# EdwardLiuyc/StaticMapping

Measured on AMD Instinct MI355X. Metric: scan-pair alignments/sec (120k-pt KITTI-64, 20 ICP iters), higher is better.
Workload: dtype f32/f64; 1 GPU; BASELINE config #2: IcpFast point-to-plane, 120k-pt synthetic Velodyne-64 scan pair vs CalculateNormals target (~21695 pts), exactly 20 iterations, rho 0.7; 512 distinct consecutive pairs of a synthetic drive (speed 6-10 m/s, yaw rate +-0.2 rad/s, seed 5), guess = previous pair's motion; pairs_per_gpu=512, distinct_pairs=512, target_points_mean=21695, nn_mode=grid, guess=extrapolated, split_after=2, parallelism=pairs round-robin over 1 GPU(s), one RCCL gather of poses, rccl_ranks=1

## Files before the change

staticmapping_amd/csrc/icp_kernels.hip:

```cpp
#include <type_traits>
#include "smhip_device.h"
#include "kd_median_tree.h"
#include "grid_lookup.h"
#include "icp_tail_math.h"

namespace smhip {

__device__ __forceinline__ bool xcd_block(int nblk, int npairs, int b_pair_base, int& pair, int& blk) {
  const int id = blockIdx.x;
  const int j = id >> 3;
  const int local = (j / nblk) * 8 + (id & 7);
  pair = b_pair_base + local;
  blk = j % nblk;
  return local < npairs;
}

__global__ __launch_bounds__(256) void tgt_reduce(IcpDev b) {
  const int pair = b.pair_base + blockIdx.y;
  const int nt = b.in[pair].nt;
  const float4* tp = b.tgt_p + (size_t)pair * b.nt_cap;
  double sx = 0, sy = 0, sz = 0;
  float mn[3] = {INFINITY, INFINITY, INFINITY}, mx[3] = {-INFINITY, -INFINITY, -INFINITY};
  const int chunk = (nt + gridDim.x - 1) / gridDim.x;
  const int lo = blockIdx.x * chunk, hi = min(nt, lo + chunk);
// ... 485 lines not shown
__device__ __forceinline__ int wave_max_i(int v) {
  constexpr int kId = -0x7fffffff - 1;
  v = max(v, dpp_or<0x111, 0xf>(kId, v));
  v = max(v, dpp_or<0x112, 0xf>(kId, v));
  v = max(v, dpp_or<0x114, 0xf>(kId, v));
  v = max(v, dpp_or<0x118, 0xf>(kId, v));
  v = max(v, dpp_or<0x142, 0xa>(kId, v));
  v = max(v, dpp_or<0x143, 0xc>(kId, v));
  return __builtin_amdgcn_readlane(v, 63);
}

__device__ __forceinline__ void search_row(const uint2* __restrict__ words, const uint32_t* __restrict__ cstart,
                                           const float4* __restrict__ tq, int rowbase, int xa, int xb,
                                           float qx, float qy, float qz, Best& best);

__device__ __forceinline__ float search_radius2(float r2cap, float dub2, float margin) {
  const float r = sqrtf(dub2) + margin;
  return fminf(r2cap, r * r);
}
__device__ __forceinline__ float search_margin(float delta) { return fminf(fmaxf(3.0f * delta, 0.01f), 0.10f); }

__global__ __launch_bounds__(kNnThreads) void nn_ball(IcpDev b, int nblk) {
  int pair, blk;
  if (!xcd_block(nblk, b.npairs, b.pair_base, pair, blk)) return;
  PairState* st = &b.state[pair];
  if (st->done) return;
  const int count = st->ns;
  const int base0 = blk * (kNnThreads * kBallItems);
  if (base0 >= count) return;
  __shared__ uint32_t s_hist[kHistBins];
  for (int k = threadIdx.x; k < kHistBins; k += kNnThreads) s_hist[k] = 0;
  __syncthreads();
  const int lane = threadIdx.x & 63;
  const size_t so = (size_t)pair * b.ns_cap;
  const uint2* __restrict__ words = b.words + (size_t)pair * kMaxGridWords;
  const uint32_t* __restrict__ cstart = b.cstart + (size_t)pair * (b.nt_cap + 1);
  const float4* __restrict__ tq = b.tq + (size_t)pair * b.nt_cap;
  const float ox = st->origin[0], oy = st->origin[1], oz = st->origin[2];
  const float h = st->h, inv_h = st->inv_h;
  const int nx = st->nx, ny = st->ny, nz = st->nz, wx = st->wx;
  const float r2cap = st->rcap2;
  const bool have_prev = st->iter > 0;
  const Pot pot = {(float)st->pot_a, (float)st->pot_b, 0.f, 0.f};
  uint32_t min_lb = 0xffffffffu;

  for (int it = 0; it < kBallItems; ++it) {
    const int e = base0 + it * kNnThreads + threadIdx.x;
    bool hard = false;
    int i = -1;
    if (e < count) {
      i = e;
      double px, py, pz;
      const float4 s4 = ld_src(b, so + i);
      transform_point(st->M, s4, px, py, pz);
      const float qx = (float)px, qy = (float)py, qz = (float)pz;
      Best best = {INFINITY, -1, INFINITY};
      float d2out = INFINITY, lbout = 0.f;
      int jout = -1;
      if (isfinite(qx) && isfinite(qy) && isfinite(qz)) {
        float R2 = r2cap;
        int jp = -1;
        if (have_prev) {
          jp = b.idx[so + i];
          if (jp >= 0) {
            double ux, uy, uz;
            transform_point(st->M_prev, s4, ux, uy, uz);
            const float ex = qx - (float)ux, ey = qy - (float)uy, ez = qz - (float)uz;
            R2 = search_radius2(r2cap, dist2(tq[jp], qx, qy, qz), search_margin(sqrtf(fmaf(ez, ez, fmaf(ey, ey, ex * ex)))));
          }
        }
        const float Rs = sqrtf(R2) * 1.0001f + 1.0e-3f * h;
        const int x0 = max(cell_coord(qx - Rs, ox, inv_h), 0), x1 = min(cell_coord(qx + Rs, ox, inv_h), nx - 1);
        const int y0 = max(cell_coord(qy - Rs, oy, inv_h), 0), y1 = min(cell_coord(qy + Rs, oy, inv_h), ny - 1);
        const int z0 = max(cell_coord(qz - Rs, oz, inv_h), 0), z1 = min(cell_coord(qz + Rs, oz, inv_h), nz - 1);
        if (x0 <= x1) {
          const float slack = 2.0e-3f * h;
          for (int z = z0; z <= z1; ++z) {
            const float zl = oz + (float)z * h;
            const float dz = fmaxf(fmaxf(zl - qz, qz - (zl + h)) - slack, 0.f);
            for (int y = y0; y <= y1; ++y) {
              const float yl = oy + (float)y * h;
              const float dy = fmaxf(fmaxf(yl - qy, qy - (yl + h)) - slack, 0.f);
              if (fmaf(dy, dy, dz * dz) > R2) continue;
              uint32_t sb, se;
              row_slots(words, (z * ny + y) * wx, x0, x1, sb, se);
              if (se > sb) {
                const uint32_t j0 = cstart[sb], j1 = cstart[se];
                for (uint32_t j = j0; j < j1; ++j) test_ascending_ru(tq[j], (int)j, qx, qy, qz, best);
              }
            }
          }
        }
        if (best.d2 <= R2) {
          d2out = best.d2;
          jout = best.j;
          lbout = sqrtf(fminf(best.s2, R2));
        } else {
          d2out = R2;
          jout = best.j >= 0 ? best.j : jp;
          lbout = -sqrtf(R2);
          hard = true;
          min_lb = min(min_lb, __float_as_uint(R2));
        }
      }
      b.d2[so + i] = d2out;
      st_match(b, so + i, jout, with_pot(lbout, pot_at(pot, norm3(s4.x, s4.y, s4.z))));
      const uint32_t key = __float_as_uint(d2out);
      if (key < 0x7f800000u) atomicAdd(&s_hist[key >> kHistShift], 1u);
    }
    const unsigned long long hm = __ballot(hard);
    if (hm) {
      uint32_t basepos = 0;
      if (lane == 0) basepos = atomicAdd(&st->hard_count, (uint32_t)__popcll(hm));
      basepos = (uint32_t)__builtin_amdgcn_readlane((int)basepos, 0);
      if (hard) b.hlist[so + basepos + __popcll(hm & ((1ull << lane) - 1ull))] = i;
    }
  }
  if (min_lb != 0xffffffffu) atomicMin(&st->min_lb_key, min_lb);
  __syncthreads();
  uint32_t* gh = b.hist + (size_t)pair * kHistBins;
  for (int k = threadIdx.x; k < kHistBins; k += kNnThreads) {
    const uint32_t v = s_hist[k];
    if (v) atomicAdd(&gh[k], v);
  }
}


__device__ __forceinline__ int nabo_class(uint32_t buckets) { return buckets <= 2u ? 0 : (buckets <= 4u ? 1 : (buckets <= 7u ? 2 : 3)); }
__device__ __forceinline__ int32_t* nabo_list_slot(const IcpDev& b, size_t so, int c, uint32_t k) {
  int32_t* base = (c < 2 ? b.dlist : b.hlist) + so;
  return (c & 1) ? base + (b.ns_cap - 1) - k : base + k;
}

template <int ITEMS>
__device__ __forceinline__ void nabo_list_append(const IcpDev& b, PairState* st, size_t so, int base, int ns, uint32_t nabo_failed, int lane) {
  static_assert(ITEMS <= 32, "one bit per round");
  if (!__ballot(nabo_failed != 0u)) return;
  unsigned long long cls2 = 0;
#pragma unroll
  for (int it = 0; it < ITEMS; ++it) {
    const int i = base + it * kNnThreads + (int)threadIdx.x;
    const uint32_t w = (nabo_failed >> it) & 1u ? (uint32_t)b.nabo_work[so + min(i, ns - 1)] : 0u;
    cls2 |= (unsigned long long)nabo_class(w) << (2 * it);
  }
  uint32_t tot[4] = {0, 0, 0, 0};
  const unsigned long long lt = (1ull << lane) - 1ull;
  auto class_masks = [&](int it, unsigned long long* m) {
    const bool f = (nabo_failed >> it) & 1u;
    const uint32_t c = (uint32_t)(cls2 >> (2 * it)) & 3u;
    const unsigned long long fm = __ballot(f), b0 = __ballot(f && (c & 1u)), b1 = __ballot(f && (c & 2u));
    m[0] = fm & ~b0 & ~b1; m[1] = fm & b0 & ~b1; m[2] = fm & ~b0 & b1; m[3] = fm & b0 & b1;
    return fm;
  };
#pragma unroll
  for (int it = 0; it < ITEMS; ++it) {
    unsigned long long m[4];
    if (!class_masks(it, m)) continue;
#pragma unroll
    for (int c = 0; c < 4; ++c) tot[c] += (uint32_t)__popcll(m[c]);
  }
  uint32_t basepos[4];
#pragma unroll
  for (int c = 0; c < 4; ++c) {
    uint32_t v = 0;
    if (lane == 0 && tot[c]) v = atomicAdd(&st->nabo_count[c], tot[c]);
    basepos[c] = (uint32_t)__builtin_amdgcn_readlane((int)v, 0);
  }
#pragma unroll
  for (int it = 0; it < ITEMS; ++it) {
    unsigned long long m[4];
    if (!class_masks(it, m)) continue;
    const uint32_t c = (uint32_t)(cls2 >> (2 * it)) & 3u;
    if ((nabo_failed >> it) & 1u) {
      const unsigned long long mine = c == 0 ? m[0] : (c == 1 ? m[1] : (c == 2 ? m[2] : m[3]));
      const uint32_t bp = c == 0 ? basepos[0] : (c == 1 ? basepos[1] : (c == 2 ? basepos[2] : basepos[3]));
      *nabo_list_slot(b, so, (int)c, bp + (uint32_t)__popcll(mine & lt)) = base + it * kNnThreads + (int)threadIdx.x;
    }
#pragma unroll
    for (int c2 = 0; c2 < 4; ++c2) basepos[c2] += (uint32_t)__popcll(m[c2]);
  }
}

template <int ITEMS, bool NABO = false>
__global__ __launch_bounds__(kNnThreads) void nn_certify(IcpDev b, int nblk) {
  int pair, blk;
  if (!xcd_block(nblk, b.npairs, b.pair_base, pair, blk)) return;
  PairState* st = &b.state[pair];
  if (st->done) return;
  const int ns = st->ns;
  const int base = blk * (kNnThreads * ITEMS);
  if (base >= ns) return;
  double Mc[12];
#pragma unroll
  for (int k = 0; k < 12; ++k) Mc[k] = st->M[k];
  const Pot pot = {(float)st->pot_a, (float)st->pot_b, 0.f, 0.f};
  __shared__ uint32_t s_hist[kHistBins];
  for (int k = threadIdx.x; k < kHistBins; k += kNnThreads) s_hist[k] = 0;
  __syncthreads();
  const int lane = threadIdx.x & 63;
  const size_t so = (size_t)pair * b.ns_cap;
  const float4* __restrict__ tq = b.tq + (size_t)pair * b.nt_cap;
  const float r_need = 0.9f * sqrtf(st->rcap2);
  uint32_t min_lb = 0xffffffffu;
  uint32_t nabo_failed = 0;
  int ic = min(base + (int)threadIdx.x, ns - 1);
  float4 s_1 = ld_src(b, so + ic);
  float l_1 = ld_lb(b, so + ic);
  int j_1 = b.idx[so + ic];
  ic = min(base + kNnThreads + (int)threadIdx.x, ns - 1);
  float4 s_2 = ld_src(b, so + ic);
  float l_2 = ld_lb(b, so + ic);
  int j_2 = b.idx[so + ic];
  float4 t_1 = tq[max(j_1, 0)];
  for (int it = 0; it < ITEMS; ++it) {
    const int i = base + it * kNnThreads + threadIdx.x;
    bool hard = false, fail = false;
    const float4 s = s_1;
    const float l = l_1;
    const int j = j_1;
    const float4 t = t_1;
    s_1 = s_2; l_1 = l_2; j_1 = j_2;
    if (it + 1 < ITEMS) t_1 = tq[max(j_1, 0)];
    if (it + 2 < ITEMS) {
      ic = min(i + 2 * kNnThreads, ns - 1);
      s_2 = ld_src(b, so + ic);
      l_2 = ld_lb(b, so + ic);
      j_2 = b.idx[so + ic];
    }
    if (i < ns) {
      double px, py, pz;
      transform_point(Mc, s, px, py, pz);
      const float qx = (float)px, qy = (float)py, qz = (float)pz;
      const float Lp = bound_now(l, pot_at(pot, norm3(s.x, s.y, s.z)));
      fail = true;
      if (NABO) {
        const float Pn = pot_at(pot, norm3(s.x, s.y, s.z));
        if (isfinite(qx) && isfinite(qy) && isfinite(qz) && l > 0.f && j >= 0 &&
            l - Pn - 4.0e-7f * (l + Pn) - 1.3e-7f * (fabsf(qx) + fabsf(qy) + fabsf(qz)) > 0.f) {
          const float d1 = dist2(t, qx, qy, qz);
          b.d2[so + i] = d1;
          atomicAdd(&s_hist[__float_as_uint(d1) >> kHistShift], 1u);
          fail = false;
        }
      } else if (isfinite(qx) && isfinite(qy) && isfinite(qz) && Lp > 0.f) {
        if (l > 0.f && j >= 0) {
          const float d1 = dist2(t, qx, qy, qz);
          if (d1 < Lp * Lp) {
            b.d2[so + i] = d1;
            atomicAdd(&s_hist[__float_as_uint(d1) >> kHistShift], 1u);
            fail = false;
          }
        } else if (l < 0.f && Lp >= r_need) {
          const float lb2 = Lp * Lp;
          b.d2[so + i] = lb2;
          atomicAdd(&s_hist[__float_as_uint(lb2) >> kHistShift], 1u);
          min_lb = min(min_lb, __float_as_uint(lb2));
          hard = true;
          fail = false;
        }
      }
    }
    const unsigned long long dm = __ballot(fail);
    if (NABO) {
      if (fail) nabo_failed |= 1u << it;
    } else if (dm) {
      uint32_t basepos = 0;
      if (lane == 0) basepos = atomicAdd(&st->deferred_count, (uint32_t)__popcll(dm));
      basepos = (uint32_t)__builtin_amdgcn_readlane((int)basepos, 0);
      if (fail) b.dlist[so + basepos + __popcll(dm & ((1ull << lane) - 1ull))] = i;
    }
    const unsigned long long hm = __ballot(hard);
    if (hm) {
      uint32_t basepos = 0;
      if (lane == 0) basepos = atomicAdd(&st->hard_count, (uint32_t)__popcll(hm));
      basepos = (uint32_t)__builtin_amdgcn_readlane((int)basepos, 0);
      if (hard) b.hlist[so + basepos + __popcll(hm & ((1ull << lane) - 1ull))] = i;
    }
  }
  if (NABO) nabo_list_append<ITEMS>(b, st, so, base, ns, nabo_failed, lane);
#pragma unroll
  for (int off = 32; off > 0; off >>= 1) min_lb = min(min_lb, (uint32_t)__shfl_xor((int)min_lb, off, 64));
  if (lane == 0 && min_lb != 0xffffffffu) atomicMin(&st->min_lb_key, min_lb);
  __syncthreads();
  uint32_t* gh = b.hist + (size_t)pair * kHistBins;
  for (int k = threadIdx.x; k < kHistBins; k += kNnThreads) {
    const uint32_t v = s_hist[k];
    if (v) atomicAdd(&gh[k], v);
  }
}

__device__ __forceinline__ void sweep_run(const float4* __restrict__ tq, uint32_t j0, uint32_t j1,
                                          float qx, float qy, float qz, Best& best) {
  uint32_t j = j0;
  for (; j + 4 <= j1; j += 4) {
    const float4 t0 = tq[j], t1 = tq[j + 1], t2 = tq[j + 2], t3 = tq[j + 3];
    test_ascending_ru(t0, (int)j, qx, qy, qz, best);
    test_ascending_ru(t1, (int)j + 1, qx, qy, qz, best);
    test_ascending_ru(t2, (int)j + 2, qx, qy, qz, best);
    test_ascending_ru(t3, (int)j + 3, qx, qy, qz, best);
  }
  for (; j < j1; ++j) test_ascending_ru(tq[j], (int)j, qx, qy, qz, best);
}

#ifndef SMHIP_PHASE_TIMING
#define SMHIP_PHASE_TIMING 0
#endif
#if SMHIP_PHASE_TIMING
#define SMHIP_PHASE(k) do { if (timing) { const unsigned long long now_ = __builtin_readcyclecounter(); tacc[k] += now_ - tprev; tprev = now_; } } while (0)
__device__ __forceinline__ unsigned long long* phase_counter(const IcpDev& b, int k) {
  return reinterpret_cast<unsigned long long*>(b.tpart) + (k / 7) * 16 + 9 + (k % 7);
}
#else
#define SMHIP_PHASE(k) do { } while (0)
#endif
template <int ITEMS, bool FIRST>
__device__ __forceinline__ void ball_lds_rounds(const IcpDev& b, PairState* st, const PairState* ls, int pair, int base0, const double* Mc,
                                                uint32_t* s_hist, uint32_t& min_lb) {
  const int ns = ls->ns;
  const Pot pot = {(float)ls->pot_a, (float)ls->pot_b, (float)ls->step_a, (float)ls->step_b};
  const float Mtx = (float)Mc[3], Mty = (float)Mc[7], Mtz = (float)Mc[11];
#if SMHIP_PHASE_TIMING
  const bool timing = (b.debug_flags & 16) != 0;
  unsigned long long tacc[14] = {0, 0, 0, 0, 0, 0, 0, 0, 0, 0, 0, 0, 0, 0};
  unsigned long long tprev = timing ? __builtin_readcyclecounter() : 0ull;
#endif
  __shared__ uint32_t s_tab[kLdsTableCap];
  __shared__ float4 s_pts[kLdsPointCap];
  __shared__ uint32_t s_roff[kLdsRowCap + 1];
  __shared__ uint32_t s_occ[kLdsRowCap / 32 + 1];
  __shared__ uint32_t s_w[17];
  __shared__ int s_box[2][6];
  float4* s_e = nullptr;
  uint16_t* s_slot = nullptr;
  uint32_t* s_nsearch = nullptr;
  if constexpr (!FIRST) {
    __shared__ float4 s_e_[ITEMS * kNnThreads];
    __shared__ uint16_t s_slot_[ITEMS * kNnThreads];
    __shared__ uint32_t s_nsearch_;
    s_e = s_e_; s_slot = s_slot_; s_nsearch = &s_nsearch_;
    if (threadIdx.x == 6) s_nsearch_ = 0;
  }
  if (threadIdx.x < 6) { s_box[0][threadIdx.x] = threadIdx.x < 3 ? 0x3fffffff : -0x3fffffff; s_box[1][threadIdx.x] = s_box[0][threadIdx.x]; }
  __syncthreads();
  const int lane = threadIdx.x & 63;
  const size_t so = (size_t)pair * b.ns_cap;
  const uint2* __restrict__ words = b.words + (size_t)pair * kMaxGridWords;
  const uint32_t* __restrict__ cstart = b.cstart + (size_t)pair * (b.nt_cap + 1);
  const float4* __restrict__ tq = b.tq + (size_t)pair * b.nt_cap;
  const float ox = ls->origin[0], oy = ls->origin[1], oz = ls->origin[2];
  const float h = ls->h, inv_h = ls->inv_h;
  const int nx = ls->nx, ny = ls->ny, nz = ls->nz, wx = ls->wx, nw = ls->nw;
  const float r2cap = ls->rcap2;
  const float r_need = 0.9f * sqrtf(r2cap);
  const bool have_prev = !FIRST && ls->iter > 0;
  const bool certify = have_prev && b.certify;

  int i = base0 + threadIdx.x;
  float4 s_cur = make_float4(0, 0, 0, 0);
  int jp_cur = -1;
  float l_cur = 0.f;
  if (i < ns) {
    s_cur = ld_src(b, so + i);
    if (have_prev) { jp_cur = b.idx[so + i]; if (certify) l_cur = ld_lb(b, so + i); }
  }

  auto query_round = [&](const int it, float& qx, float& qy, float& qz, bool& valid) -> bool {
    const int base = base0 + it * kNnThreads;
    if (base >= ns) return false;
    i = base + threadIdx.x;
    const int i_next = i + kNnThreads;
    float4 s_next = make_float4(0, 0, 0, 0);
    int jp_next = -1;
    float l_next = 0.f;
    if (it + 1 < ITEMS && i_next < ns) {
      s_next = ld_src(b, so + i_next);
      if (have_prev) { jp_next = b.idx[so + i_next]; if (certify) l_next = ld_lb(b, so + i_next); }
    }
    SMHIP_PHASE(0);
    qx = 0.f; qy = 0.f; qz = 0.f;
    valid = false;
    if (i < ns) {
      double px, py, pz;
      transform_point(Mc, s_cur, px, py, pz);
      qx = (float)px; qy = (float)py; qz = (float)pz;
      valid = isfinite(qx) && isfinite(qy) && isfinite(qz);
    }
    const bool has_jp = valid && jp_cur >= 0;
    float dub2 = INFINITY;
    if (has_jp) dub2 = dist2(tq[jp_cur], qx, qy, qz);
    bool need_search = valid, hard = false;
    if (i < ns && !valid) {
      b.d2[so + i] = INFINITY; st_match(b, so + i, -1, 0.f);
    }
    const float sn = __builtin_amdgcn_sqrtf(fmaf(s_cur.z, s_cur.z, fmaf(s_cur.y, s_cur.y, s_cur.x * s_cur.x)));
    const float delta = have_prev ? fmaf(pot.sa, sn, pot.sb) : 0.03f;
    if (certify && valid) {
      const float Lp = bound_now(l_cur, pot_at(pot, sn));
      if (Lp > 0.f) {
        if (l_cur > 0.f && has_jp && dub2 < Lp * Lp) {
          b.d2[so + i] = dub2;
          atomicAdd(&s_hist[__float_as_uint(dub2) >> kHistShift], 1u);
          need_search = false;
        } else if (l_cur < 0.f && Lp >= r_need) {
          const float lb2 = Lp * Lp;
          b.d2[so + i] = lb2;
          atomicAdd(&s_hist[__float_as_uint(lb2) >> kHistShift], 1u);
          min_lb = min(min_lb, __float_as_uint(lb2));
          hard = true;
          need_search = false;
        }
      }
    }
    if constexpr (!FIRST) {
      const unsigned long long sm = __ballot(need_search);
      if (sm) {
        uint32_t basepos = 0;
        if (lane == 0) basepos = atomicAdd(s_nsearch, (uint32_t)__popcll(sm));
        basepos = (uint32_t)__builtin_amdgcn_readlane((int)basepos, 0);
        if (need_search) {
          const uint32_t pos = basepos + __popcll(sm & ((1ull << lane) - 1ull));
          s_e[pos] = make_float4(qx, qy, qz, has_jp ? search_radius2(r2cap, dub2, search_margin(delta)) : r2cap);
          s_slot[pos] = (uint16_t)(it * kNnThreads + (int)threadIdx.x);
        }
      }
    }
    {
      const unsigned long long hm = __ballot(hard);
      if (hm) {
        uint32_t basepos = 0;
        if (lane == 0) basepos = atomicAdd(&st->hard_count, (uint32_t)__popcll(hm));
        basepos = (uint32_t)__builtin_amdgcn_readlane((int)basepos, 0);
        if (hard) b.hlist[so + basepos + __popcll(hm & ((1ull << lane) - 1ull))] = i;
      }
    }
    s_cur = s_next; jp_cur = jp_next; l_cur = l_next;
    SMHIP_PHASE(1);
    return true;
  };
  auto search_round = [&](const int sr, const bool mine, const bool wave_live, const float qx, const float qy, const float qz, const float R2, const int gi) {
    int* box = s_box[sr & 1];
#if SMHIP_PHASE_TIMING
    const unsigned long long tround = timing ? __builtin_readcyclecounter() : 0ull;
#endif
    int x0 = 1, x1 = 0, y0 = 1, y1 = 0, z0 = 1, z1 = 0;
    if (mine) {
      const float Rs = __builtin_amdgcn_sqrtf(R2) * 1.0001f + 1.0e-3f * h;
      x0 = max(cell_coord(qx - Rs, ox, inv_h), 0); x1 = min(cell_coord(qx + Rs, ox, inv_h), nx - 1);
      y0 = max(cell_coord(qy - Rs, oy, inv_h), 0); y1 = min(cell_coord(qy + Rs, oy, inv_h), ny - 1);
      z0 = max(cell_coord(qz - Rs, oz, inv_h), 0); z1 = min(cell_coord(qz + Rs, oz, inv_h), nz - 1);
    }
    const bool inbox = mine && x0 <= x1 && y0 <= y1 && z0 <= z1;
    if (wave_live) {
      const int big = 0x3fffffff;
      const int mx0 = wave_min_i(inbox ? x0 : big), mx1 = wave_max_i(inbox ? x1 : -big);
      const int my0 = wave_min_i(inbox ? y0 : big), my1 = wave_max_i(inbox ? y1 : -big);
      const int mz0 = wave_min_i(inbox ? z0 : big), mz1 = wave_max_i(inbox ? z1 : -big);
      if (lane == 0 && mx0 <= mx1) {
        atomicMin(&box[0], mx0); atomicMin(&box[1], my0); atomicMin(&box[2], mz0);
        atomicMax(&box[3], mx1); atomicMax(&box[4], my1); atomicMax(&box[5], mz1);
      }
    }
    SMHIP_PHASE(3);
    __syncthreads();
    const int X0 = box[0], Y0 = box[1], Z0 = box[2];
    const int nxl = box[3] - X0 + 2, nyl = box[4] - Y0 + 1, nzl = box[5] - Z0 + 1;
    const bool any = box[3] >= X0;
    const long long entries = any ? (long long)nxl * nyl * nzl : 0;
    const bool use_lds = any && entries <= kLdsTableCap;
    if (use_lds) {
      const float inv_nxl = 1.0f / (float)nxl, inv_nyl = 1.0f / (float)nyl;
      for (int e = threadIdx.x; e < (int)entries; e += kNnThreads) {
        const int r = (int)(((float)e + 0.5f) * inv_nxl);
        const int x = X0 + (e - r * nxl);
        const int zz = (int)(((float)r + 0.5f) * inv_nyl);
        const int y = Y0 + (r - zz * nyl), z = Z0 + zz;
        const int widx = (z * ny + y) * wx + (x >> 5);
        uint32_t val = (uint32_t)ls->nt;
        if (widx < nw) {
          const uint2 wd = words[widx];
          val = cstart[wd.y + __popc(wd.x & ((1u << (x & 31)) - 1u))];
        }
        s_tab[e] = val;
      }
    }
    if (threadIdx.x < 6) s_box[(sr + 1) & 1][threadIdx.x] = threadIdx.x < 3 ? 0x3fffffff : -0x3fffffff;
    const int rows = use_lds ? nyl * nzl : 0;
    bool pts_lds = use_lds && rows <= kLdsRowCap;
    if (use_lds) __syncthreads();
    if (pts_lds) {
      uint32_t len = 0;
      if ((int)threadIdx.x < rows) len = s_tab[threadIdx.x * nxl + nxl - 1] - s_tab[threadIdx.x * nxl];
      {
        const unsigned long long om = __ballot(len > 0);
        if (lane == 0) { s_occ[2 * (threadIdx.x >> 6)] = (uint32_t)om; s_occ[2 * (threadIdx.x >> 6) + 1] = (uint32_t)(om >> 32); }
        if (threadIdx.x == 0) s_occ[kLdsRowCap / 32] = 0u;
      }
      uint32_t total;
      const uint32_t off = block_excl_scan(len, s_w, &total);
      if ((int)threadIdx.x < rows) s_roff[threadIdx.x] = off;
      if (threadIdx.x == 0) s_roff[rows] = total;
      __syncthreads();
      pts_lds = total <= (uint32_t)kLdsPointCap;
      if (pts_lds) {
        for (uint32_t k = threadIdx.x; k < total; k += kNnThreads) {
          int lo = 0, hi = rows - 1;
          while (lo < hi) { const int mid = (lo + hi + 1) >> 1; if (s_roff[mid] <= k) lo = mid; else hi = mid - 1; }
          const uint32_t j = s_tab[lo * nxl] + (k - s_roff[lo]);
          float4 t = tq[j];
          t.w = __int_as_float((int)j);
          s_pts[k] = t;
        }
      }
    }
    __syncthreads();
    SMHIP_PHASE(4);
    bool hard2 = false;
    if (mine) {
      Best best = {INFINITY, -1, INFINITY};
      if (x0 <= x1 && y0 <= y1 && z0 <= z1) {
        const float slack = 2.0e-3f * h;
        const uint32_t ymask = (2u << (y1 - y0)) - 1u;
        for (int z = z0; z <= z1; ++z) {
          const float zl = oz + (float)z * h;
          const float dz = fmaxf(fmaxf(zl - qz, qz - (zl + h)) - slack, 0.f);
          const int ra = (z - Z0) * nyl + (y0 - Y0);
          uint32_t m = ymask;
          if (pts_lds) m &= __builtin_amdgcn_alignbit(s_occ[(ra >> 5) + 1], s_occ[ra >> 5], (uint32_t)(ra & 31));
          while (m) {
            const int bpos = __ffs((int)m) - 1;
            m &= m - 1u;
            const int y = y0 + bpos;
            const float yl = oy + (float)y * h;
            const float dy = fmaxf(fmaxf(yl - qy, qy - (yl + h)) - slack, 0.f);
            if (fmaf(dy, dy, dz * dz) > R2) continue;
            if (pts_lds) {
              const int r = ra + bpos;
              const int rb = r * nxl - X0;
              const uint32_t g0 = s_tab[rb + X0];
              const uint32_t k0 = s_roff[r] + (s_tab[rb + x0] - g0), k1 = s_roff[r] + (s_tab[rb + x1 + 1] - g0);
              for (const float4 *tp = s_pts + k0, *te = s_pts + k1; tp < te; ++tp) {
                const float4 t = *tp;
                test_ascending_ru(t, __float_as_int(t.w), qx, qy, qz, best);
              }
            } else if (use_lds) {
              const int rb = (ra + bpos) * nxl - X0;
              sweep_run(tq, s_tab[rb + x0], s_tab[rb + x1 + 1], qx, qy, qz, best);
            } else {
              uint32_t sb, se;
              row_slots(words, (z * ny + y) * wx, x0, x1, sb, se);
              if (se > sb) sweep_run(tq, cstart[sb], cstart[se], qx, qy, qz, best);
            }
          }
        }
      }
      float d2out, lbout;
      int jout;
      if (best.d2 <= R2) {
        d2out = best.d2;
        jout = best.j;
        lbout = __builtin_amdgcn_sqrtf(fminf(best.s2, R2));
      } else {
        d2out = R2;
        jout = best.j >= 0 ? best.j : (have_prev ? b.idx[so + gi] : -1);
        lbout = -__builtin_amdgcn_sqrtf(R2);
        hard2 = true;
        min_lb = min(min_lb, __float_as_uint(R2));
      }
      SMHIP_PHASE(5);
      b.d2[so + gi] = d2out;
      {
        const float ux = qx - Mtx, uy = qy - Mty, uz = qz - Mtz;
        st_match(b, so + gi, jout, with_pot(lbout, pot_at(pot, __builtin_amdgcn_sqrtf(fmaf(uz, uz, fmaf(uy, uy, ux * ux))))));
      }
      const uint32_t key = __float_as_uint(d2out);
      if (key < 0x7f800000u) atomicAdd(&s_hist[key >> kHistShift], 1u);
    }
    {
      const unsigned long long hm = __ballot(hard2);
      if (hm) {
        uint32_t basepos = 0;
        if (lane == 0) basepos = atomicAdd(&st->hard_count, (uint32_t)__popcll(hm));
        basepos = (uint32_t)__builtin_amdgcn_readlane((int)basepos, 0);
        if (hard2) b.hlist[so + basepos + __popcll(hm & ((1ull << lane) - 1ull))] = gi;
      }
    }
    SMHIP_PHASE(6);
#if SMHIP_PHASE_TIMING
    if (timing) {
      const unsigned long long dt = __builtin_readcyclecounter() - tround, one = threadIdx.x < 64 ? 1ull : 0ull;
      if (pts_lds) { tacc[8] += one; tacc[9] += dt; }
      else if (use_lds) { tacc[10] += one; tacc[11] += dt; }
      else { tacc[12] += one; tacc[13] += dt; }
    }
#endif
  };
  if constexpr (FIRST) {
    uint32_t nvalid = 0;
    for (int it = 0; it < ITEMS; ++it) {
      float qx, qy, qz;
      bool valid;
      if (!query_round(it, qx, qy, qz, valid)) break;
      const unsigned long long vm = __ballot(valid);
      nvalid += (uint32_t)__popcll(vm);
      SMHIP_PHASE(2);
      search_round(it, valid, vm != 0ull, qx, qy, qz, r2cap, base0 + it * kNnThreads + (int)threadIdx.x);
    }
    if (lane == 0 && nvalid) atomicAdd(&st->deferred_count, nvalid);
  } else {
    for (int it = 0; it < ITEMS; ++it) {
      float qx, qy, qz;
      bool valid;
      if (!query_round(it, qx, qy, qz, valid)) break;
    }
    __syncthreads();
    SMHIP_PHASE(2);
    const int nq = (int)*s_nsearch;
    if (threadIdx.x == 0 && nq) atomicAdd(&st->deferred_count, (uint32_t)nq);
    for (int sr = 0, e0 = 0; e0 < nq; ++sr, e0 += kNnThreads) {
      const int e = e0 + (int)threadIdx.x;
      const bool mine = e < nq;
      float4 q4 = make_float4(0.f, 0.f, 0.f, 0.f);
      int gi = -1;
      if (mine) { q4 = s_e[e]; gi = base0 + (int)s_slot[e]; }
      search_round(sr, mine, (e & ~63) < nq, q4.x, q4.y, q4.z, q4.w, gi);
    }
  }
#if SMHIP_PHASE_TIMING
  if (timing && lane == 0) {
    for (int k = 0; k < 14; ++k) atomicAdd(phase_counter(b, k), tacc[k]);
  }
#endif
}

__device__ __forceinline__ void flush_min_lb(PairState* st, uint32_t min_lb) {
#pragma unroll
  for (int off = 32; off > 0; off >>= 1) min_lb = min(min_lb, (uint32_t)__shfl_xor((int)min_lb, off, 64));
  if ((threadIdx.x & 63) == 0 && min_lb != 0xffffffffu) atomicMin(&st->min_lb_key, min_lb);
}
__device__ __forceinline__ void flush_hist(const IcpDev& b, int pair, const uint32_t* s_hist) {
  __syncthreads();
  uint32_t* gh = b.hist + (size_t)pair * kHistBins;
  for (int k = threadIdx.x; k < kHistBins; k += kNnThreads) {
    const uint32_t v = s_hist[k];
    if (v) atomicAdd(&gh[k], v);
  }
}
__device__ __forceinline__ void flush_min_lb_and_hist(const IcpDev& b, PairState* st, int pair, uint32_t min_lb, const uint32_t* s_hist) {
  flush_min_lb(st, min_lb);
  flush_hist(b, pair, s_hist);
}

template <int ITEMS, bool FIRST = false>
__global__ __launch_bounds__(kNnThreads, 5) void nn_ball_lds(IcpDev b, int nblk) {
  int pair, blk;
  if (!xcd_block(nblk, b.npairs, b.pair_base, pair, blk)) return;
  PairState* st = &b.state[pair];
  if (st->done) return;
  const int base0 = blk * (kNnThreads * ITEMS);
  if (base0 >= st->ns) return;
  double Mc[12];
#pragma unroll
  for (int k = 0; k < 12; ++k) Mc[k] = st->M[k];
  __shared__ uint32_t s_hist[kHistBins];
  for (int k = threadIdx.x; k < kHistBins; k += kNnThreads) s_hist[k] = 0;
  uint32_t min_lb = 0xffffffffu;
  ball_lds_rounds<ITEMS, FIRST>(b, st, st, pair, base0, Mc, s_hist, min_lb);
  flush_min_lb_and_hist(b, st, pair, min_lb, s_hist);
}

__device__ __forceinline__ void listed_append_hard(const IcpDev& b, PairState* st, size_t so, bool hard, int i, int lane);
constexpr int kWaveBoxRows = 1024;
constexpr int kWaveCand = 256;

__device__ __forceinline__ void lane_ball_search(const uint2* __restrict__ words, const uint32_t* __restrict__ cstart, const float4* __restrict__ tq,
                                                 float ox, float oy, float oz, float h, int ny, int wx, float qx, float qy, float qz, float R2,
                                                 int x0, int x1, int y0, int y1, int z0, int z1, Best& best) {
  const float slack = 2.0e-3f * h;
  for (int z = z0; z <= z1; ++z) {
    const float zl = oz + (float)z * h;
    const float dz = fmaxf(fmaxf(zl - qz, qz - (zl + h)) - slack, 0.f);
    for (int y = y0; y <= y1; ++y) {
      const float yl = oy + (float)y * h;
      const float dy = fmaxf(fmaxf(yl - qy, qy - (yl + h)) - slack, 0.f);
      if (fmaf(dy, dy, dz * dz) > R2) continue;
      uint32_t sb, se;
      row_slots(words, (z * ny + y) * wx, x0, x1, sb, se);
      if (se > sb) {
        const uint32_t j0 = cstart[sb], j1 = cstart[se];
        for (uint32_t j = j0; j < j1; ++j) test_ascending_ru(tq[j], (int)j, qx, qy, qz, best);
      }
    }
  }
}
__device__ __forceinline__ void test_pair_ru(const float4 a, const float4 c, float qx, float qy, float qz, Best& best) {
  const f32x2 dx = (f32x2){qx, qx} - (f32x2){a.x, a.y};
  const f32x2 dy = (f32x2){qy, qy} - (f32x2){a.z, a.w};
  const f32x2 dz = (f32x2){qz, qz} - (f32x2){c.x, c.y};
  f32x2 d = dx * dx;
  d = __builtin_elementwise_fma(dy, dy, d);
  d = __builtin_elementwise_fma(dz, dz, d);
  best.s2 = __builtin_amdgcn_fmed3f(d.x, best.d2, best.s2);
  if (d.x < best.d2) { best.d2 = d.x; best.j = __float_as_int(c.z); }
  best.s2 = __builtin_amdgcn_fmed3f(d.y, best.d2, best.s2);
  if (d.y < best.d2) { best.d2 = d.y; best.j = __float_as_int(c.w); }
}

template <int ITEMS, bool FIRST>
__global__ __launch_bounds__(kNnThreads) void nn_ball_wave(IcpDev b, int nblk) {
  int pair, blk;
  if (!xcd_block(nblk, b.npairs, b.pair_base, pair, blk)) return;
  PairState* st = &b.state[pair];
  if (st->done) return;
  const int ns = st->ns;
  const int base0 = blk * (kNnThreads * ITEMS);
  if (base0 >= ns) return;
  double Mc[12];
#pragma unroll
  for (int k = 0; k < 12; ++k) Mc[k] = st->M[k];
  const Pot pot = {(float)st->pot_a, (float)st->pot_b, (float)st->step_a, (float)st->step_b};
  const float Mtx = (float)Mc[3], Mty = (float)Mc[7], Mtz = (float)Mc[11];
  __shared__ uint32_t s_hist[kHistBins];
  __shared__ float4 s_cand[kNnThreads / 64][kWaveCand];
  __shared__ uint32_t s_roff[kNnThreads / 64][64];
  __shared__ uint32_t s_rbase[kNnThreads / 64][64];
  __shared__ uint32_t s_nsearch;
  for (int k = threadIdx.x; k < kHistBins; k += kNnThreads) s_hist[k] = 0;
  if (threadIdx.x == 0) s_nsearch = 0;
  __syncthreads();
  const int lane = threadIdx.x & 63, wave = threadIdx.x >> 6;
  float4* cand = s_cand[wave];
  uint32_t* roff = s_roff[wave];
  uint32_t* rbase = s_rbase[wave];
  const size_t so = (size_t)pair * b.ns_cap;
  const uint2* __restrict__ words = b.words + (size_t)pair * kMaxGridWords;
  const uint32_t* __restrict__ cstart = b.cstart + (size_t)pair * (b.nt_cap + 1);
  const float4* __restrict__ tq = b.tq + (size_t)pair * b.nt_cap;
  const float ox = st->origin[0], oy = st->origin[1], oz = st->origin[2];
  const float h = st->h, inv_h = st->inv_h;
  const int nx = st->nx, ny = st->ny, nz = st->nz, wx = st->wx;
  const float r2cap = st->rcap2;
  const float r_need = 0.9f * sqrtf(r2cap);
  const bool have_prev = !FIRST && st->iter > 0;
  const bool certify = have_prev && b.certify;
  uint32_t min_lb = 0xffffffffu;
  uint32_t nsearch = 0;

  int i = base0 + threadIdx.x;
  float4 s_cur = make_float4(0, 0, 0, 0);
  int jp_cur = -1;
  float l_cur = 0.f;
  if (i < ns) {
    s_cur = ld_src(b, so + i);
    if (have_prev) { jp_cur = b.idx[so + i]; if (certify) l_cur = ld_lb(b, so + i); }
  }
  for (int it = 0; it < ITEMS; ++it) {
    const int base = base0 + it * kNnThreads;
    if (base >= ns) break;
    i = base + threadIdx.x;
    const int i_next = i + kNnThreads;
    float4 s_next = make_float4(0, 0, 0, 0);
    int jp_next = -1;
    float l_next = 0.f;
    if (it + 1 < ITEMS && i_next < ns) {
      s_next = ld_src(b, so + i_next);
      if (have_prev) { jp_next = b.idx[so + i_next]; if (certify) l_next = ld_lb(b, so + i_next); }
    }
    float qx = 0.f, qy = 0.f, qz = 0.f;
    bool valid = false;
    if (i < ns) {
      double px, py, pz;
      transform_point(Mc, s_cur, px, py, pz);
      qx = (float)px; qy = (float)py; qz = (float)pz;
      valid = isfinite(qx) && isfinite(qy) && isfinite(qz);
    }
    const bool has_jp = valid && jp_cur >= 0;
    float dub2 = INFINITY;
    if (has_jp) dub2 = dist2(tq[jp_cur], qx, qy, qz);
    bool need_search = valid, hard = false;
    if (i < ns && !valid) {
      b.d2[so + i] = INFINITY; st_match(b, so + i, -1, 0.f);
    }
    float R2 = r2cap;
    if (!FIRST) {
      const float sn = __builtin_amdgcn_sqrtf(fmaf(s_cur.z, s_cur.z, fmaf(s_cur.y, s_cur.y, s_cur.x * s_cur.x)));
      const float delta = have_prev ? fmaf(pot.sa, sn, pot.sb) : 0.03f;
      if (certify && valid) {
        const float Lp = bound_now(l_cur, pot_at(pot, sn));
        if (Lp > 0.f) {
          if (l_cur > 0.f && has_jp && dub2 < Lp * Lp) {
            b.d2[so + i] = dub2;
            atomicAdd(&s_hist[__float_as_uint(dub2) >> kHistShift], 1u);
            need_search = false;
          } else if (l_cur < 0.f && Lp >= r_need) {
            const float lb2 = Lp * Lp;
            b.d2[so + i] = lb2;
            atomicAdd(&s_hist[__float_as_uint(lb2) >> kHistShift], 1u);
            min_lb = min(min_lb, __float_as_uint(lb2));
            hard = true;
            need_search = false;
          }
        }
      }
      if (has_jp) R2 = search_radius2(r2cap, dub2, search_margin(delta));
      listed_append_hard(b, st, so, hard, i, lane);
    }
    const unsigned long long sm = __ballot(need_search);
    if (sm) {
      nsearch += (uint32_t)__popcll(sm);
      int x0 = 1, x1 = 0, y0 = 1, y1 = 0, z0 = 1, z1 = 0;
      if (need_search) {
        const float Rs = __builtin_amdgcn_sqrtf(R2) * 1.0001f + 1.0e-3f * h;
        x0 = max(cell_coord(qx - Rs, ox, inv_h), 0); x1 = min(cell_coord(qx + Rs, ox, inv_h), nx - 1);
        y0 = max(cell_coord(qy - Rs, oy, inv_h), 0); y1 = min(cell_coord(qy + Rs, oy, inv_h), ny - 1);
        z0 = max(cell_coord(qz - Rs, oz, inv_h), 0); z1 = min(cell_coord(qz + Rs, oz, inv_h), nz - 1);
      }
      const bool inbox = need_search && x0 <= x1 && y0 <= y1 && z0 <= z1;
      const int big = 0x3fffffff;
      const int X0 = wave_min_i(inbox ? x0 : big), X1 = wave_max_i(inbox ? x1 : -big);
      const int Y0 = wave_min_i(inbox ? y0 : big), Y1 = wave_max_i(inbox ? y1 : -big);
      const int Z0 = wave_min_i(inbox ? z0 : big), Z1 = wave_max_i(inbox ? z1 : -big);
      Best best = {INFINITY, -1, INFINITY};
      if (X0 <= X1) {
        const int nyl = Y1 - Y0 + 1;
        const long long nrows_ll = (long long)nyl * (Z1 - Z0 + 1);
        if (nrows_ll <= kWaveBoxRows) {
          const int nrows = (int)nrows_ll;
          const float inv_nyl = 1.0f / (float)nyl;
          for (int r0 = 0; r0 < nrows; r0 += 64) {
            const int r = r0 + lane;
            uint32_t j0 = 0, len = 0;
            if (r < nrows) {
              const int zz = (int)(((float)r + 0.5f) * inv_nyl);
              const int y = Y0 + (r - zz * nyl), z = Z0 + zz;
              uint32_t sb, se;
              row_slots(words, (z * ny + y) * wx, X0, X1, sb, se);
              if (se > sb) { j0 = cstart[sb]; len = cstart[se] - j0; }
            }
            const uint32_t incl = wave_incl_scan(len, lane);
            const int N = __builtin_amdgcn_readlane((int)incl, 63);
            if (N == 0) continue;
            roff[lane] = incl - len;
            rbase[lane] = j0 - (incl - len);
            __builtin_amdgcn_fence(__ATOMIC_RELEASE, "wavefront");
            __builtin_amdgcn_wave_barrier();
            for (int p0 = 0; p0 < N; p0 += kWaveCand) {
              const int cnt = min(kWaveCand, N - p0);
#pragma unroll
              for (int m = 0; m < kWaveCand / 64; ++m) {
                if (64 * m >= cnt) break;
                const int c = lane + 64 * m;
                const uint32_t k = (uint32_t)(p0 + min(c, cnt - 1));
                int rho = 0;
#pragma unroll
                for (int step = 32; step > 0; step >>= 1) rho = roff[min(rho + step, 63)] <= k && rho + step < 64 ? rho + step : rho;
                const uint32_t j = rbase[rho] + k;
                const float4 t = tq[j];
                if (c < cnt) {
                  float* o = reinterpret_cast<float*>(cand + 2 * (c >> 1)) + (c & 1);
                  o[0] = t.x; o[2] = t.y; o[4] = t.z; o[6] = __int_as_float((int)j);
                }
              }
              if ((cnt & 1) && lane == 0) {
                float* o = reinterpret_cast<float*>(cand + 2 * (cnt >> 1)) + 1;
                o[0] = 3.0e38f; o[2] = 0.f; o[4] = 0.f; o[6] = __int_as_float(-1);
              }
              __builtin_amdgcn_fence(__ATOMIC_RELEASE, "wavefront");
              __builtin_amdgcn_wave_barrier();
              const int npair = (cnt + 1) >> 1;
#pragma unroll 4
              for (int pp = 0; pp < npair; ++pp) test_pair_ru(cand[2 * pp], cand[2 * pp + 1], qx, qy, qz, best);
              __builtin_amdgcn_fence(__ATOMIC_RELEASE, "wavefront");
              __builtin_amdgcn_wave_barrier();
            }
          }
        } else if (inbox) {
          lane_ball_search(words, cstart, tq, ox, oy, oz, h, ny, wx, qx, qy, qz, R2, x0, x1, y0, y1, z0, z1, best);
        }
      }
      bool hard2 = false;
      if (need_search) {
        float d2out, lbout;
        int jout;
        if (best.d2 <= R2) {
          d2out = best.d2;
          jout = best.j;
          lbout = __builtin_amdgcn_sqrtf(fminf(best.s2, R2));
        } else {
          d2out = R2;
          jout = best.j >= 0 ? best.j : jp_cur;
          lbout = -__builtin_amdgcn_sqrtf(R2);
          hard2 = true;
          min_lb = min(min_lb, __float_as_uint(R2));
        }
        b.d2[so + i] = d2out;
        {
          const float ux = qx - Mtx, uy = qy - Mty, uz = qz - Mtz;
          st_match(b, so + i, jout, with_pot(lbout, pot_at(pot, __builtin_amdgcn_sqrtf(fmaf(uz, uz, fmaf(uy, uy, ux * ux))))));
        }
        const uint32_t key = __float_as_uint(d2out);
        if (key < 0x7f800000u) atomicAdd(&s_hist[key >> kHistShift], 1u);
      }
      listed_append_hard(b, st, so, hard2, i, lane);
    }
    s_cur = s_next; jp_cur = jp_next; l_cur = l_next;
  }
  if (lane == 0 && nsearch) atomicAdd(&s_nsearch, nsearch);
#pragma unroll
  for (int off = 32; off > 0; off >>= 1) min_lb = min(min_lb, (uint32_t)__shfl_xor((int)min_lb, off, 64));
  if (lane == 0 && min_lb != 0xffffffffu) atomicMin(&st->min_lb_key, min_lb);
  __syncthreads();
  if (threadIdx.x == 0 && s_nsearch) atomicAdd(&st->deferred_count, s_nsearch);
  uint32_t* gh = b.hist + (size_t)pair * kHistBins;
  for (int k = threadIdx.x; k < kHistBins; k += kNnThreads) {
    const uint32_t v = s_hist[k];
    if (v) atomicAdd(&gh[k], v);
  }
}

__device__ __forceinline__ void sweep_run_any(const float4* __restrict__ tq, uint32_t j0, uint32_t j1,
                                              float qx, float qy, float qz, Best& best) {
  uint32_t j = j0;
  for (; j + 4 <= j1; j += 4) {
    const float4 t0 = tq[j], t1 = tq[j + 1], t2 = tq[j + 2], t3 = tq[j + 3];
    test_any_order(t0, (int)j, qx, qy, qz, best);
    test_any_order(t1, (int)j + 1, qx, qy, qz, best);
    test_any_order(t2, (int)j + 2, qx, qy, qz, best);
    test_any_order(t3, (int)j + 3, qx, qy, qz, best);
  }
  for (; j < j1; ++j) test_any_order(tq[j], (int)j, qx, qy, qz, best);
}

__device__ __forceinline__ void search_row(const uint2* __restrict__ words, const uint32_t* __restrict__ cstart,
                                           const float4* __restrict__ tq, int rowbase, int xa, int xb,
                                           float qx, float qy, float qz, Best& best) {
  uint32_t sb, se;
  row_slots(words, rowbase, xa, xb, sb, se);
  if (se > sb) {
    sweep_run_any(tq, cstart[sb], cstart[se], qx, qy, qz, best);
  }
}

__device__ __forceinline__ bool ring_irrelevant(const IcpDev& b, float g, float best_d2) {
  return b.nn_cutoff2 > 0.f && g * g >= b.nn_cutoff2 && best_d2 >= b.nn_cutoff2;
}

__device__ __forceinline__ bool ring_search_query(const IcpDev& b, const PairState* st, int pair, float qx, float qy, float qz, Best& best) {
  bool resolved = true;
  if (isfinite(qx) && isfinite(qy) && isfinite(qz)) {
    const uint2* words = b.words + (size_t)pair * kMaxGridWords;
    const uint32_t* cstart = b.cstart + (size_t)pair * (b.nt_cap + 1);
    const float4* tq = b.tq + (size_t)pair * b.nt_cap;
    const float ox = st->origin[0], oy = st->origin[1], oz = st->origin[2];
    const float inv_h = st->inv_h;
    const int nx = st->nx, ny = st->ny, nz = st->nz, wx = st->wx;
    const int cx = cell_coord(qx, ox, inv_h), cy = cell_coord(qy, oy, inv_h), cz = cell_coord(qz, oz, inv_h);
    int rp = 0;
    resolved = false;
    for (int r = 1; r <= b.max_ring; r *= 2) {
// ... 1875 lines not shown
```

staticmapping_amd/csrc/smhip_device.h:

```cpp
#pragma once

#include <hip/hip_runtime.h>
#include <stdint.h>

namespace smhip {

constexpr int kHistBins = 2048;
constexpr int kHistShift = 20;
constexpr int kSearchHist = 12;
constexpr int kNnThreads = 256;
constexpr int kAccThreads = 256;
constexpr int kAccItemsSmall = 8;
constexpr int kAccItemsBatch = 32;
constexpr int kFinalizeKeyCap = 8192;
constexpr int kFinalizeMaxSeg = 2048;
constexpr int kScoreParts = 16;
constexpr int kAccCols = 32;
constexpr int kMaxGridWords = 1 << 18;
constexpr int kMaxRowWords = (kMaxGridWords >> 5) + 2;
constexpr int kTgtReduceBlocks = 32;
constexpr int kBruteTile = 1024;
constexpr int kFallbackSlices = 64;
constexpr int kLdsTableCap = 1024;
constexpr int kLdsPointCap = 512;
constexpr int kLdsRowCap = 256;
constexpr int kWideBlocks = 512;
constexpr int kNaboAccBlocks = 8;
constexpr int kListedMaxPairs = 1024;
constexpr int kListedItemBlocks = 1280;
constexpr int kListedBlocks = 32;
constexpr int kBallItems = 2;
constexpr int kListedLaneBudgetMax = 32768;
constexpr int kFusedListedMax = 16384;
constexpr int kListedMaxItems = (kFusedListedMax / kNnThreads > kListedLaneBudgetMax / kNnThreads ? kFusedListedMax / kNnThreads : kListedLaneBudgetMax / kNnThreads) + 1;
constexpr int kListedSumChunk = 4096;
constexpr int kSumsBlocks = 2048;
constexpr int kCertifyItems = 32;

constexpr int kOneMaxRounds = 16;
constexpr int kOneSyncWords = 4096;
constexpr int kOneMaxBlocks = 1024;
constexpr int kOnePairs = 8;

struct PairState {
  double M[12];
  double M_prev[12];
  double pot_a, pot_b;
  double step_a, step_b;
  double T_iter[16];
  double G[16];
  double mu[3];
  double guess[16];
  double quat[5][4];
  double trans[5][3];
  int32_t n_hist;
  int32_t iter;
  int32_t done;
  int32_t status;
  int32_t ns;
  int32_t nt;
  int32_t has_normals;
  float origin[3];
  float h;
  float inv_h;
  int32_t nx, ny, nz, wx, nw;
  int32_t nocc;
  uint32_t unresolved_count;
  uint32_t fallback_ticket;
  uint32_t fallback_total;
  uint32_t searched_total;
  uint32_t deferred_count;
  uint32_t hard_count;
  uint32_t hard_total;
  uint32_t min_lb_key;
  int32_t refine;
  uint32_t refine_total;
  float rcap2;
  int32_t kept;
  uint32_t limit_key;
  uint32_t nabo_count[4];
  int32_t grid_invalid;
  int32_t band_lo, band_hi;
  int32_t spec_ok;
  uint32_t spec_hits;
  uint32_t listed_ticket;
  uint32_t pad2_;

  double score_part[kScoreParts];
  uint32_t score_cnt[kScoreParts];
  uint32_t score_mismatch;
  uint32_t pad_score_;
  double score;
  double result[16];
};

struct PairInput {
  double guess[16];
  int32_t ns;
  int32_t nt;
  int32_t has_normals;
  int32_t pad;
};

struct IcpDev {
  int32_t slots, ns_cap, nt_cap;
  int32_t npairs;
  int32_t pair_base;
  int32_t acc_blocks;
  int32_t part_stride;
  int32_t bl_stride;
  int32_t dl_stride;
  int32_t seg_stride;
  int32_t fused;
  float band_pad;
  int32_t fused_nabo;
  int32_t listed_lane_budget;
  int32_t listed_grain;
  float band_gain;
  int32_t acc_items;
  int32_t sums_items;
  PairState* state;
  const PairInput* in;
  const float4* src;
  const float* src3;
  const float4* tgt_p;
  const float4* tgt_n;
  float4* tq;
  float4* tn;
  uint32_t* tcell;
  uint32_t* tslot;
  uint32_t* tord;
  uint32_t* bits;
  uint2* words;
  uint32_t* rowbits;
  int32_t have_rowbits;
  uint32_t* ccount;
  uint32_t* cstart;
  float* lb;
  float* d2;
  int32_t* idx;
  uint32_t* mb;
  uint32_t* hist;
  int32_t* dlist;
  int32_t* hlist;
  int32_t* ulist;
  unsigned long long* ukeys;
  float4* rec_a;
  int32_t* rec_j;
  uint32_t* gcount;
  int32_t* dcount;
  uint32_t* litems;
  double* partials;
  double* tpart;
  uint32_t* done_count;
  uint32_t* one_sync;
  double* one_rows;
  uint32_t* one_hist;
  uint32_t* one_keys;
  PairState* one_ctr;
  uint8_t* nabo_work;
  uint32_t* search_hist;
  int32_t max_iteration;
  int32_t early_exit;
  int32_t max_ring;
  float nn_cutoff2;
  int32_t sort_cells;
  int32_t use_ball;
  int32_t lds_table;
  int32_t certify;
  int32_t split_after;
  int32_t exact_all;
  float ball_radius;
  float cap_factor;
  float rho;
  float grid_cell;
  int32_t debug_flags;
  float* comp3;
};

}
```

Baseline: 28000 alignments/s.

## Batch global-grid row sweeps and enlarge first-round LDS point cache

Replaces the per-row global grid sweep with a batched routine that fetches occupancy words and cstart ranges for four rows at once, then walks their concatenated point runs in groups of four. The aim is to overlap independent global loads and reduce divergent per-row loop overhead. It also gives the FIRST variant a larger LDS point cache with a higher occupancy launch bound, and marks pair/blk as wave-uniform via readfirstlane. The extra LDS and register pressure could reduce occupancy, and the bigger cache only helps when a ball's points fit in it.

```diff
diff --git a/staticmapping_amd/csrc/icp_kernels.hip b/staticmapping_amd/csrc/icp_kernels.hip
--- a/staticmapping_amd/csrc/icp_kernels.hip
+++ b/staticmapping_amd/csrc/icp_kernels.hip
@@ -811,6 +811,55 @@
   for (; j < j1; ++j) test_ascending_ru(tq[j], (int)j, qx, qy, qz, best);
 }
 
+__device__ __forceinline__ uint32_t run_pos(uint32_t c, uint32_t e0, uint32_t e1, uint32_t e2, uint32_t o0, uint32_t o1, uint32_t o2, uint32_t o3) {
+  return c + (c < e0 ? o0 : c < e1 ? o1 : c < e2 ? o2 : o3);
+}
+__device__ __forceinline__ void sweep_rows_global(const uint2* __restrict__ words, const uint32_t* __restrict__ cstart, const float4* __restrict__ tq,
+                                                  int ny, int wx, float oy, float oz, float h, float slack, int x0, int x1, int y0, int y1, int z0, int z1,
+                                                  float qx, float qy, float qz, float R2, Best& best) {
+  const int wa_i = x0 >> 5, wc_i = x1 >> 5;
+  const bool two = wa_i != wc_i;
+  const uint32_t ma = (1u << (x0 & 31)) - 1u, mc = 0xffffffffu >> (31 - (x1 & 31));
+  int y = y0, z = z0;
+  while (z <= z1) {
+    uint2 wa[4], wc[4];
+#pragma unroll
+    for (int k = 0; k < 4; ++k) {
+      const float zl = oz + (float)z * h, yl = oy + (float)y * h;
+      const float dz = fmaxf(fmaxf(zl - qz, qz - (zl + h)) - slack, 0.f);
+      const float dy = fmaxf(fmaxf(yl - qy, qy - (yl + h)) - slack, 0.f);
+      wa[k] = make_uint2(0u, 0u); wc[k] = make_uint2(0u, 0u);
+      if (z <= z1 && !(fmaf(dy, dy, dz * dz) > R2)) {
+        const int rowbase = (z * ny + y) * wx;
+        wa[k] = words[rowbase + wa_i];
+        if (two) wc[k] = words[rowbase + wc_i];
+      }
+      if (++y > y1) { y = y0; ++z; }
+    }
+    uint32_t j0[4], j1[4];
+#pragma unroll
+    for (int k = 0; k < 4; ++k) {
+      const uint2 c = two ? wc[k] : wa[k];
+      const uint32_t sb = wa[k].y + __popc(wa[k].x & ma), se = c.y + __popc(c.x & mc);
+      j0[k] = 0u; j1[k] = 0u;
+      if (se > sb) { j0[k] = cstart[sb]; j1[k] = cstart[se]; }
+    }
+    const uint32_t e0 = j1[0] - j0[0], e1 = e0 + (j1[1] - j0[1]), e2 = e1 + (j1[2] - j0[2]), tot = e2 + (j1[3] - j0[3]);
+    const uint32_t o0 = j0[0], o1 = j0[1] - e0, o2 = j0[2] - e1, o3 = j0[3] - e2;
+    for (uint32_t c = 0u; c < tot; c += 4) {
+      const uint32_t e = tot - 1u;
+      const uint32_t cb = min(c + 1u, e), cc = min(c + 2u, e), cd = min(c + 3u, e);
+      const uint32_t ja = run_pos(c, e0, e1, e2, o0, o1, o2, o3), jb = run_pos(cb, e0, e1, e2, o0, o1, o2, o3);
+      const uint32_t jc = run_pos(cc, e0, e1, e2, o0, o1, o2, o3), jd = run_pos(cd, e0, e1, e2, o0, o1, o2, o3);
+      const float4 a0 = tq[ja], a1 = tq[jb], a2 = tq[jc], a3 = tq[jd];
+      test_ascending_ru(a0, (int)ja, qx, qy, qz, best);
+      if (c + 1u <= e) test_ascending_ru(a1, (int)jb, qx, qy, qz, best);
+      if (c + 2u <= e) test_ascending_ru(a2, (int)jc, qx, qy, qz, best);
+      if (c + 3u <= e) test_ascending_ru(a3, (int)jd, qx, qy, qz, best);
+    }
+  }
+}
+
 #ifndef SMHIP_PHASE_TIMING
 #define SMHIP_PHASE_TIMING 0
 #endif
@@ -834,7 +883,8 @@
   unsigned long long tprev = timing ? __builtin_readcyclecounter() : 0ull;
 #endif
   __shared__ uint32_t s_tab[kLdsTableCap];
-  __shared__ float4 s_pts[kLdsPointCap];
+  constexpr int kPointCap = FIRST ? kLdsPointCapFirst : kLdsPointCap;
+  __shared__ float4 s_pts[kPointCap];
   __shared__ uint32_t s_roff[kLdsRowCap + 1];
   __shared__ uint32_t s_occ[kLdsRowCap / 32 + 1];
   __shared__ uint32_t s_w[17];
@@ -1001,7 +1051,7 @@
       if ((int)threadIdx.x < rows) len = s_tab[threadIdx.x * nxl + nxl - 1] - s_tab[threadIdx.x * nxl];
       {
         const unsigned long long om = __ballot(len > 0);
-        if (lane == 0) { s_occ[2 * (threadIdx.x >> 6)] = (uint32_t)om; s_occ[2 * (threadIdx.x >> 6) + 1] = (uint32_t)(om >> 32); }
+        if (lane == 0) { const int w2 = 2 * __builtin_amdgcn_readfirstlane((int)(threadIdx.x >> 6)); s_occ[w2] = (uint32_t)om; s_occ[w2 + 1] = (uint32_t)(om >> 32); }
         if (threadIdx.x == 0) s_occ[kLdsRowCap / 32] = 0u;
       }
       uint32_t total;
@@ -1009,7 +1059,7 @@
       if ((int)threadIdx.x < rows) s_roff[threadIdx.x] = off;
       if (threadIdx.x == 0) s_roff[rows] = total;
       __syncthreads();
-      pts_lds = total <= (uint32_t)kLdsPointCap;
+      pts_lds = total <= (uint32_t)kPointCap;
       if (pts_lds) {
         for (uint32_t k = threadIdx.x; k < total; k += kNnThreads) {
           int lo = 0, hi = rows - 1;
@@ -1028,8 +1078,9 @@
       Best best = {INFINITY, -1, INFINITY};
       if (x0 <= x1 && y0 <= y1 && z0 <= z1) {
         const float slack = 2.0e-3f * h;
-        const uint32_t ymask = (2u << (y1 - y0)) - 1u;
-        for (int z = z0; z <= z1; ++z) {
+        if (!use_lds) sweep_rows_global(words, cstart, tq, ny, wx, oy, oz, h, slack, x0, x1, y0, y1, z0, z1, qx, qy, qz, R2, best);
+        else for (int z = z0; z <= z1; ++z) {
+          const uint32_t ymask = (2u << (y1 - y0)) - 1u;
           const float zl = oz + (float)z * h;
           const float dz = fmaxf(fmaxf(zl - qz, qz - (zl + h)) - slack, 0.f);
           const int ra = (z - Z0) * nyl + (y0 - Y0);
@@ -1051,13 +1102,9 @@
                 const float4 t = *tp;
                 test_ascending_ru(t, __float_as_int(t.w), qx, qy, qz, best);
               }
-            } else if (use_lds) {
+            } else {
               const int rb = (ra + bpos) * nxl - X0;
               sweep_run(tq, s_tab[rb + x0], s_tab[rb + x1 + 1], qx, qy, qz, best);
-            } else {
-              uint32_t sb, se;
-              row_slots(words, (z * ny + y) * wx, x0, x1, sb, se);
-              if (se > sb) sweep_run(tq, cstart[sb], cstart[se], qx, qy, qz, best);
             }
           }
         }
@@ -1160,9 +1207,10 @@
 }
 
 template <int ITEMS, bool FIRST = false>
-__global__ __launch_bounds__(kNnThreads, 5) void nn_ball_lds(IcpDev b, int nblk) {
+__global__ __launch_bounds__(kNnThreads, FIRST ? 6 : 5) void nn_ball_lds(IcpDev b, int nblk) {
   int pair, blk;
   if (!xcd_block(nblk, b.npairs, b.pair_base, pair, blk)) return;
+  pair = __builtin_amdgcn_readfirstlane(pair); blk = __builtin_amdgcn_readfirstlane(blk);
   PairState* st = &b.state[pair];
   if (st->done) return;
   const int base0 = blk * (kNnThreads * ITEMS);
diff --git a/staticmapping_amd/csrc/smhip_device.h b/staticmapping_amd/csrc/smhip_device.h
--- a/staticmapping_amd/csrc/smhip_device.h
+++ b/staticmapping_amd/csrc/smhip_device.h
@@ -23,6 +23,7 @@
 constexpr int kFallbackSlices = 64;
 constexpr int kLdsTableCap = 1024;
 constexpr int kLdsPointCap = 512;
+constexpr int kLdsPointCapFirst = 768;
 constexpr int kLdsRowCap = 256;
 constexpr int kWideBlocks = 512;
 constexpr int kNaboAccBlocks = 8;
```

After: 29000 alignments/s (median of 6 runs). 3.6% higher.
